# mnigm2001/Software-Defined-Radio

Hardware: AMD Instinct MI355X
Metric: I/Q MS/s through front-end FIR+decimate+demod(+audio) per job; % HBM roofline (higher is better)
Workload: dtype i8+f32

## Files before the change

### software-defined-radio_amd/csrc/kernels_fe_mfma.hip

```cpp
#include "device_math.hpp"
#include "fe_mfma_host.hpp"
#include "fmrx_internal.hpp"

#include <cmath>
#include <type_traits>
#include <utility>

namespace fmrx {
namespace {

using i4 = int __attribute__((ext_vector_type(4)));
using f2 = float __attribute__((ext_vector_type(2)));
using f4 = float __attribute__((ext_vector_type(4)));

constexpr int kNtPolicy = 2;

constexpr int iclamp(int v, int lo, int hi) { return v < lo ? lo : (v > hi ? hi : v); }
constexpr int igcd(int a, int b) { return b == 0 ? a : igcd(b, a % b); }

template <int T, int D, int PF = 0>
struct MfCfg {
    static constexpr int COL_OUT = 8;
    static constexpr int COLS = 16;
    static constexpr int TILE_OUT = COL_OUT * (COLS - 1);
// ... 210 lines not shown
        for (int d = 0; d < C::NDIG; d++) acc[d] = (i4){0, 0, 0, 0};
#pragma unroll
        for (int j = 0; j < C::KSTEPS; j++) {
            const i4 bs = b[j] ^ static_cast<int>(0x80808080u);
#pragma unroll
            for (int d = 0; d < C::NDIG; d++) acc[d] = __builtin_amdgcn_mfma_i32_16x16x64_i8(a[j][d], bs, acc[d], 0, 0, 0);
        }

        float v[4];
#pragma unroll
        for (int k = 0; k < 4; k++) {
            int lo = acc[0][k];
            if (C::NDIG >= 2) lo += acc[1][k] * 256;
            const float flo = static_cast<float>(lo) * scale_lo;
            v[k] = C::NDIG >= 3 ? __builtin_fmaf(static_cast<float>(acc[2][k]), scale_hi, flo) : flo;
        }
        float pi = __shfl(v[2], src_lane, 64), pq = __shfl(v[3], src_lane, 64);
        const long o = static_cast<long>(tile) * C::TILE_OUT + C::COL_OUT * (col - 1) + 2 * g;
        if (override_prev && o == 0) {
            pi = ovi;
            pq = ovq;
        }
        float d0 = 0.0f, d1 = 0.0f;
        if (demod) {
            d0 = demod_fast(v[0], v[1], pi, pq);
            d1 = demod_fast(v[2], v[3], v[0], v[1]);
        }

        if (col > 0 && o < n_out) {
            if (o + 1 < n_out) {
                if (demod) *reinterpret_cast<f2 *>(demod + o) = (f2){d0, d1};
                if (with_if) *reinterpret_cast<f4 *>(y_if + 2 * o) = (f4){v[0], v[1], v[2], v[3]};
                if (prev_out && o + 2 == n_out) *prev_out = make_float2(v[2], v[3]);
            } else {
                if (demod) demod[o] = d0;
                if (with_if) *reinterpret_cast<f2 *>(y_if + 2 * o) = (f2){v[0], v[1]};
                if (prev_out) *prev_out = make_float2(v[0], v[1]);
            }
        }
        slot = slot + 1 == C::NSLOT ? 0 : slot + 1;
        fill = fill + 1 == C::NSLOT ? 0 : fill + 1;
    }
}

template <int T, int D, int MINB = 2, int PF = 0>
int launch_mfma(const FePlan &pl, const uint8_t *d_iq, size_t n_samples, const uint8_t *d_hist, const float *d_prev,
                float *d_demod, float *d_if, float *d_prev_out, uint8_t *d_hist_next, hipStream_t stream,
                const float *d_dhist_src = nullptr, float *d_dhist_dst = nullptr, int dhist_n = 0)
{
    using C = MfCfg<T, D, PF>;
    if (C::LEAD > pl.hist_bytes) return fail(FMRX_EINVAL, "fe_mfma: history too short");
    const long n_out = static_cast<long>(n_samples / D);
    const long n_tiles = (n_out + C::TILE_OUT - 1) / C::TILE_OUT;
    long wgs_per_cu = (160 * 1024) / (4L * C::RING);
    if (wgs_per_cu > MINB) wgs_per_cu = MINB;
    const long want = (n_tiles + 3) / 4;
    const long grid = want < 256 * wgs_per_cu ? want : 256 * wgs_per_cu;
    hipLaunchKernelGGL((fe_mfma_kernel<T, D, MINB, PF>), dim3(static_cast<unsigned>(grid)), dim3(256), 4 * C::RING, stream, d_iq,
                       d_hist + pl.hist_bytes, static_cast<long>(2 * n_samples), reinterpret_cast<const i4 *>(pl.a_img.p),
                       pl.scale_lo, reinterpret_cast<const float2 *>(d_prev), d_demod, d_if,
                       reinterpret_cast<float2 *>(d_prev_out), n_out, static_cast<int>(n_tiles), d_hist_next, pl.hist_bytes,
                       d_dhist_src, d_dhist_dst, dhist_n);
    hipError_t e = hipGetLastError();
    if (e != hipSuccess) return fail(FMRX_EHIP, "launch fe_mfma_kernel<%d,%d>: %s", T, D, hipGetErrorString(e));
    return FMRX_OK;
}

struct FeBankGeom {
    long in_pitch, in_off;
    long out_pitch, out_off;
    long n_row;
    int tiles_per_row;
};

template <int T, int D>
__global__ __launch_bounds__(256, 2) void fe_mfma_bank_kernel(const uint8_t *__restrict__ x, long n_bytes, const i4 *__restrict__ a_img,
                                                               float scale_lo, float *__restrict__ demod, FeBankGeom bk, int n_tiles)
{
    using C = MfCfg<T, D, 0>;
    extern __shared__ __attribute__((aligned(16))) uint8_t lds_raw[];
    const int lane = threadIdx.x & 63;
    const int wave = __builtin_amdgcn_readfirstlane(static_cast<int>(threadIdx.x >> 6));
    uint8_t *ring = lds_raw + wave * C::RING;
    const int tstep = static_cast<int>(gridDim.x) * 4;
    int tile = __builtin_amdgcn_readfirstlane(static_cast<int>(blockIdx.x) * 4 + wave);
    if (tile >= n_tiles) return;
    i4 a[C::KSTEPS][C::NDIG];
#pragma unroll
    for (int j = 0; j < C::KSTEPS; j++)
#pragma unroll
        for (int d = 0; d < C::NDIG; d++) a[j][d] = a_img[(j * C::NDIG + d) * 64 + lane];
    asm volatile("s_waitcnt vmcnt(0)" ::: "memory");
#pragma unroll
    for (int j = 0; j < C::KSTEPS; j++)
#pragma unroll
        for (int d = 0; d < C::NDIG; d++) asm volatile("" : "+v"(a[j][d]));
    auto dma = [&](int t, int rs) {
        const int c = t / bk.tiles_per_row, j = t - c * bk.tiles_per_row;
        const long s0 = c * bk.in_pitch + bk.in_off + static_cast<long>(j) * C::STRIDE_BYTES - C::LEAD;
        dma_window<C::NPF, C::REM_LANES>(x, x, n_bytes, s0, ring + rs * C::SLOT, lane);
    };
#pragma unroll
    for (int k = 0; k < C::P; k++)
        if (tile + k * tstep < n_tiles) dma(tile + k * tstep, k);
    const int col = lane & 15, g = lane >> 4;
    const int lane_off = C::COL_BYTES * col + 16 * g;
    const float scale_hi = scale_lo * 65536.0f;
    const int src_lane = lane >= 16 ? lane - 16 : lane + 47;
    int slot = 0, fill = C::P;
    for (int it = 0; tile < n_tiles; tile += tstep, it++) {
        const bool steady = tile + C::P * tstep < n_tiles;
        if (steady) dma(tile + C::P * tstep, fill);
        if (steady) {
            if (it < C::P) wait_vmcnt<C::YOUNGER>();
            else wait_vmcnt<C::YOUNGER + C::P>();
        } else {
            wait_vmcnt<0>();
        }
        __builtin_amdgcn_fence(__ATOMIC_ACQUIRE, "wavefront");
        __builtin_amdgcn_wave_barrier();
        const uint8_t *bsrc = ring + slot * C::SLOT + lane_off;
        i4 b[C::KSTEPS];
#pragma unroll
        for (int j = 0; j < C::KSTEPS; j++) b[j] = *reinterpret_cast<const i4 *>(bsrc + 64 * j);
        __builtin_amdgcn_s_waitcnt(0xC07F);
        __builtin_amdgcn_fence(__ATOMIC_RELEASE, "wavefront");
        __builtin_amdgcn_wave_barrier();
        i4 acc[C::NDIG];
#pragma unroll
        for (int d = 0; d < C::NDIG; d++) acc[d] = (i4){0, 0, 0, 0};
#pragma unroll
        for (int j = 0; j < C::KSTEPS; j++) {
            const i4 bs = b[j] ^ static_cast<int>(0x80808080u);
#pragma unroll
            for (int d = 0; d < C::NDIG; d++) acc[d] = __builtin_amdgcn_mfma_i32_16x16x64_i8(a[j][d], bs, acc[d], 0, 0, 0);
        }
        float v[4];
#pragma unroll
        for (int k = 0; k < 4; k++) {
            int lo = acc[0][k];
            if (C::NDIG >= 2) lo += acc[1][k] * 256;
            const float flo = static_cast<float>(lo) * scale_lo;
            v[k] = C::NDIG >= 3 ? __builtin_fmaf(static_cast<float>(acc[2][k]), scale_hi, flo) : flo;
        }
        const float pi = __shfl(v[2], src_lane, 64), pq = __shfl(v[3], src_lane, 64);
        const float d0 = demod_fast(v[0], v[1], pi, pq), d1 = demod_fast(v[2], v[3], v[0], v[1]);
        const int c = tile / bk.tiles_per_row, j = tile - c * bk.tiles_per_row;
        const long ol = static_cast<long>(j) * C::TILE_OUT + C::COL_OUT * (col - 1) + 2 * g;
        if (col > 0 && ol < bk.n_row) *reinterpret_cast<f2 *>(demod + c * bk.out_pitch + bk.out_off + ol) = (f2){d0, d1};
        slot = slot + 1 == C::NSLOT ? 0 : slot + 1;
        fill = fill + 1 == C::NSLOT ? 0 : fill + 1;
    }
}

template <int T, int D, int TA, int DA>
struct FuCfg {
    using F = MfCfg<T, D>;
    static constexpr int TILE_OUT = 128;
    static constexpr int TILE_BYTES = F::COL_BYTES * 16;
    static constexpr int NPF = TILE_BYTES / 1024;
    static constexpr int REM_LANES = (TILE_BYTES % 1024) / 16;
    static constexpr int NP = NPF + (REM_LANES ? 1 : 0);
    static constexpr int P = iclamp(6144 / TILE_BYTES, 2, 8);
    static constexpr int NSLOT = P + 2;
    static constexpr int RING = NSLOT * TILE_BYTES;
    static constexpr int PIECE0 = NPF ? 1024 : TILE_BYTES;
    static_assert(F::WIN - F::COL_BYTES <= PIECE0, "window overlap must fit the next slot's first piece");
    static_assert(64 * F::KSTEPS - F::COL_BYTES <= RING - TILE_BYTES, "K padding laps the ring");
    static constexpr int YOUNGER = (NP - 1) + NP * P;
    static_assert(YOUNGER <= 63, "vmcnt is 6 bits");
    static constexpr int AB_OUT = 256;
    static constexpr int TB = AB_OUT * DA / TILE_OUT;
    static_assert(TB * TILE_OUT == AB_OUT * DA, "batches end on tile boundaries");
    static constexpr int SLOT_STEP = igcd(TB, NSLOT);
    static constexpr int NSTART = NSLOT / SLOT_STEP;
    static constexpr int LANE_OFF_END = F::COL_BYTES * (F::COLS - 1) + 16 * 3 + 16;
    static constexpr int AWIN = (TA - 1) + 15 * DA + 1;
    static constexpr int AK = (AWIN + 15) / 16 * 4;
    static_assert(AK % 4 == 0 && (TA - 1) % 4 == 0, "window in whole 16-byte groups");
    static constexpr int KPT = ((AK + TB - 3) / (TB - 2) + 3) / 4 * 4;
    static constexpr int NPH = (AK + KPT - 1) / KPT;
    static constexpr int DR_MIN = AB_OUT * DA + TA - 1 + (4 * AK - AWIN) + (NPH + 1) * TILE_OUT;
    static constexpr int DR = (DR_MIN + TILE_OUT - 1) / TILE_OUT * TILE_OUT;
    static_assert(NPH <= TB - 2, "a batch must be done before the next one completes");
    static_assert(AB_OUT * DA + TA - 1 + (4 * AK - AWIN) + (NPH + 1) * TILE_OUT <= DR, "ring too small for the delayed multiply");
    static_assert(DR % TILE_OUT == 0, "tiles must not wrap inside");
    static_assert(TA - 1 <= TILE_OUT - 1, "one dry tile must cover the audio history");
    static constexpr int MIRROR = 4 * KPT;
    static_assert(MIRROR <= TILE_OUT, "the mirror is refreshed by the tile at position 0");
    static constexpr int LDS_WAVE = RING + (DR + MIRROR) * 4;
};

template <class C, class F>
__device__ __forceinline__ void fu_dma_slot(const uint8_t *__restrict__ x, const uint8_t *__restrict__ hist_end, long n_bytes,
                                            int u, uint8_t *ring, int rs, int lane)
{
    dma_window<C::NPF, C::REM_LANES, kNtPolicy>(x, hist_end, n_bytes, static_cast<long>(u) * C::TILE_BYTES - F::FRONT,
                                                ring + rs * C::TILE_BYTES, lane);
}

template <int T, int D, int TA, int DA>
__global__ __launch_bounds__(256, 2) void mono_fused_kernel(
    const uint8_t *__restrict__ x, const uint8_t *__restrict__ hist_end, long n_bytes, const i4 *__restrict__ a_img,
    float scale_lo, const float *__restrict__ au_img, const float2 *__restrict__ prev_in,
    const float *__restrict__ dhist_end, float *__restrict__ demod_tail, int tail_keep, float2 *__restrict__ prev_out,
    float *__restrict__ audio, int16_t *__restrict__ pcm, int wrap, long n_out, int n_tiles, long n_audio, int n_batches,
    int batches_per_wave, uint8_t *__restrict__ hist_next, int hist_bytes)
{
    using C = FuCfg<T, D, TA, DA>;
    using F = typename C::F;
    extern __shared__ __attribute__((aligned(16))) uint8_t lds_raw[];
    const int lane = threadIdx.x & 63;
    const int wave = __builtin_amdgcn_readfirstlane(static_cast<int>(threadIdx.x >> 6));
    uint8_t *ring = lds_raw + wave * C::LDS_WAVE;
    float *dring = reinterpret_cast<float *>(ring + C::RING);
    const int wid = __builtin_amdgcn_readfirstlane(static_cast<int>(blockIdx.x) * 4 + wave);

    if (hist_next && wid == 0)
        for (int i = lane; i < hist_bytes; i += 64) hist_next[i] = x[n_bytes - hist_bytes + i];

    const int b0 = wid * batches_per_wave;
    const int b1 = b0 + batches_per_wave < n_batches ? b0 + batches_per_wave : n_batches;
    if (b0 >= b1) return;
    const int t0 = b0 * C::TB;
    const int t1 = b1 * C::TB < n_tiles ? b1 * C::TB : n_tiles;
    const int tb = t0 > 0 ? t0 - 1 : 0;

    i4 a[F::KSTEPS][F::NDIG];
#pragma unroll
    for (int j = 0; j < F::KSTEPS; j++)
#pragma unroll
        for (int d = 0; d < F::NDIG; d++) a[j][d] = a_img[(j * F::NDIG + d) * 64 + lane];
    float au[C::AK];
#pragma unroll
    for (int j = 0; j < C::AK; j++) au[j] = au_img[j * 64 + lane];
    float ci = 0.0f, cq = 0.0f;
    for (int i = lane; i < C::DR + C::MIRROR; i += 64) dring[i] = 0.0f;
    if (t0 == 0) {
        const float2 p = *prev_in;
        ci = p.x;
        cq = p.y;
        for (int i = lane; i < TA - 1; i += 64) dring[C::TILE_OUT - (TA - 1) + i] = dhist_end[i - (TA - 1)];
    }
    asm volatile("s_waitcnt vmcnt(0) lgkmcnt(0)" ::: "memory");
#pragma unroll
    for (int j = 0; j < F::KSTEPS; j++)
#pragma unroll
        for (int d = 0; d < F::NDIG; d++) asm volatile("" : "+v"(a[j][d]));
#pragma unroll
    for (int j = 0; j < C::AK; j++) asm volatile("" : "+v"(au[j]));
    asm volatile("" : "+v"(ci), "+v"(cq));

    for (int u = tb; u <= tb + C::P && u <= t1; u++) fu_dma_slot<C, F>(x, hist_end, n_bytes, u, ring, u % C::NSLOT, lane);

    const int col = lane & 15, g = lane >> 4;
    const int lane_off = F::COL_BYTES * col + 16 * g;
    const float scale_hi = scale_lo * 65536.0f;
    const int src_lane = lane >= 16 ? lane - 16 : lane + 47;
    int wrap_adr[F::KSTEPS];
#pragma unroll
    for (int j = 0; j < F::KSTEPS; j++) {
        const int adr = (C::NSLOT - 1) * C::TILE_BYTES + lane_off + 64 * j;
        wrap_adr[j] = adr >= C::RING ? adr - C::RING : adr;
    }
    int slot = tb % C::NSLOT, fill = (tb + C::P + 1) % C::NSLOT;
    int dpos = C::TILE_OUT;
    bool pend = false;
    int pend_ph = 0, pend_ws = 0;
    long pend_a0 = 0;
    f4 y0 = (f4){0.0f, 0.0f, 0.0f, 0.0f}, y1 = y0;
    f4 xs[C::KPT / 4];
    auto slice_load = [&]() {
#pragma unroll
        for (int k = 0; k < C::KPT / 4; k++)
            xs[k] = *reinterpret_cast<const f4 *>(dring + pend_ws + 16 * k);
        pend_ws += 4 * C::KPT;
        pend_ws = pend_ws >= C::DR ? pend_ws - C::DR : pend_ws;
    };
    auto slice_mfma = [&]() {
#pragma unroll
        for (int ph = 0; ph < C::NPH; ph++)
            if (pend_ph == ph) {
#pragma unroll
                for (int j = ph * C::KPT; j < (ph + 1) * C::KPT && j < C::AK; j++) {
                    const float xv = xs[(j - ph * C::KPT) / 4][j % 4];
                    if (j & 1) y1 = __builtin_amdgcn_mfma_f32_16x16x4f32(au[j], xv, y1, 0, 0, 0);
                    else y0 = __builtin_amdgcn_mfma_f32_16x16x4f32(au[j], xv, y0, 0, 0, 0);
                }
            }
    };
    auto store_batch = [&]() {
        const f4 y = y0 + y1;
        const long ao = pend_a0 + 4 * g;
        if (ao + 3 < n_audio) {
            if (audio) *reinterpret_cast<f4 *>(audio + ao) = y;
            if (pcm) {
                using s4 = short __attribute__((ext_vector_type(4)));
                const s4 pk = (s4){pcm_pack_flat(y[0], wrap), pcm_pack_flat(y[1], wrap), pcm_pack_flat(y[2], wrap), pcm_pack_flat(y[3], wrap)};
                *reinterpret_cast<s4 *>(pcm + ao) = pk;
            }
        } else {
#pragma unroll
            for (int k = 0; k < 4; k++)
                if (ao + k < n_audio) {
                    if (audio) audio[ao + k] = y[k];
                    if (pcm) pcm[ao + k] = pcm_pack(y[k], wrap);
                }
        }
    };
    auto slice_done = [&]() {
        pend_ph++;
        if (pend_ph == C::NPH) {
            store_batch();
            pend = false;
        }
    };
    auto begin_batch = [&](int bt) {
        pend = true;
        pend_ph = 0;
        pend_a0 = static_cast<long>(bt) * C::AB_OUT + 16 * col;
        int sb = (bt * C::AB_OUT * DA - (TA - 1)) - (C::TILE_OUT * tb - C::TILE_OUT);
        pend_ws = (sb + 16 * col * DA + 4 * g) % C::DR;
        y0 = (f4){0.0f, 0.0f, 0.0f, 0.0f};
        y1 = y0;
    };
    int t_fast1 = 0;
    bool fast_last = false;
    if (scale_lo >= 8.8817842e-16f) {
        const long in_x = (n_bytes - C::NP * 1024L + F::FRONT) / C::TILE_BYTES;
        const long no_tail = (n_out - tail_keep) / C::TILE_OUT - 1;
        long lim = t1 - C::P - 1;
        lim = lim < in_x - C::P - 1 ? lim : in_x - C::P - 1;
        lim = lim < no_tail ? lim : no_tail;
        t_fast1 = lim + 1 >= C::TB ? static_cast<int>((lim + 1) / C::TB) * C::TB : 0;
        fast_last = t1 % C::TB == 0 && t1 - C::TB >= t0 && t1 <= in_x && t1 - 1 <= no_tail;
    }
    int t_cur = tb;
    const long rbase = static_cast<long>(tb) * C::TILE_BYTES;
    const long reach = static_cast<long>(t1 - tb + 1) * C::TILE_BYTES + C::NP * 1024L;
    const __amdgpu_buffer_rsrc_t xr = __builtin_amdgcn_make_buffer_rsrc(
        const_cast<uint8_t *>(x + rbase), 0, static_cast<int>(reach < n_bytes - rbase ? reach : n_bytes - rbase), 0x00020000);
    const int lane16 = 16 * lane;
    const uint8_t *lring = ring + lane_off;
    auto fast_tile = [&](auto kc, auto lastc, auto sc, int t) {
        constexpr int k = decltype(kc)::value;
        constexpr int U = (decltype(sc)::value + k) % C::NSLOT;
        constexpr int FILL = (U + C::P + 1) % C::NSLOT;
        constexpr bool STEADY = !decltype(lastc)::value || k + C::P + 1 <= C::TB;
        constexpr int WAIT = STEADY ? C::YOUNGER : (C::NP - 1) + C::NP * (C::TB - k - 1);
        auto slice_k = [&]() {
#pragma unroll
            for (int j = k * C::KPT; j < (k + 1) * C::KPT && j < C::AK; j++) {
                const float xv = xs[(j - k * C::KPT) / 4][j % 4];
                if (j & 1) y1 = __builtin_amdgcn_mfma_f32_16x16x4f32(au[j], xv, y1, 0, 0, 0);
                else y0 = __builtin_amdgcn_mfma_f32_16x16x4f32(au[j], xv, y0, 0, 0, 0);
            }
        };
        if constexpr (STEADY) {
            const int soff = (t + C::P + 1 - tb) * C::TILE_BYTES - F::FRONT;
            for_each_index(std::make_integer_sequence<int, C::NP>{}, [&](auto qc) {
                constexpr int q = decltype(qc)::value;
                if (q < C::NPF || lane < C::REM_LANES)
                    __builtin_amdgcn_raw_ptr_buffer_load_lds(
                        xr, (__attribute__((address_space(3))) void *)(ring + FILL * C::TILE_BYTES + q * 1024), 16, lane16,
                        soff + q * 1024, 0, kNtPolicy);
            });
        }
        wait_vmcnt<WAIT>();
        __builtin_amdgcn_fence(__ATOMIC_ACQUIRE, "wavefront");
        __builtin_amdgcn_wave_barrier();
        i4 b[F::KSTEPS];
        for_each_index(std::make_integer_sequence<int, F::KSTEPS>{}, [&](auto jc) {
            constexpr int j = decltype(jc)::value;
            constexpr int OFF = U * C::TILE_BYTES + 64 * j;
            if constexpr (OFF + C::LANE_OFF_END > C::RING) {
                static_assert(U == C::NSLOT - 1, "only the last slot wraps");
                b[j] = *reinterpret_cast<const i4 *>(ring + wrap_adr[j]);
            } else {
                b[j] = *reinterpret_cast<const i4 *>(lring + OFF);
            }
        });
        if constexpr (k < C::NPH) slice_load();
        __builtin_amdgcn_sched_barrier(0);
        __builtin_amdgcn_s_waitcnt(0xC07F);
        __builtin_amdgcn_fence(__ATOMIC_RELEASE, "wavefront");
        __builtin_amdgcn_wave_barrier();
        i4 acc[F::NDIG];
#pragma unroll
        for (int d = 0; d < F::NDIG; d++) acc[d] = (i4){0, 0, 0, 0};
#pragma unroll
        for (int j = 0; j < F::KSTEPS; j++) {
            const i4 bs = b[j] ^ static_cast<int>(0x80808080u);
#pragma unroll
            for (int d = 0; d < F::NDIG; d++) acc[d] = __builtin_amdgcn_mfma_i32_16x16x64_i8(a[j][d], bs, acc[d], 0, 0, 0);
        }
        float v[4];
#pragma unroll
        for (int q = 0; q < 4; q++) {
            int lo = acc[0][q];
            if (F::NDIG >= 2) lo += acc[1][q] * 256;
            const float flo = static_cast<float>(lo) * scale_lo;
            v[q] = F::NDIG >= 3 ? __builtin_fmaf(static_cast<float>(acc[2][q]), scale_hi, flo) : flo;
        }
        float pi = __shfl(v[2], src_lane, 64), pq = __shfl(v[3], src_lane, 64);
        pi = lane == 0 ? ci : pi;
        pq = lane == 0 ? cq : pq;
        ci = __builtin_bit_cast(float, __builtin_amdgcn_readlane(__builtin_bit_cast(int, v[2]), 63));
        cq = __builtin_bit_cast(float, __builtin_amdgcn_readlane(__builtin_bit_cast(int, v[3]), 63));
        const float d0 = demod_fast_bounded(v[0], v[1], pi, pq);
        const float d1 = demod_fast_bounded(v[2], v[3], v[0], v[1]);
        const int ol = F::COL_OUT * col + 2 * g;
        *reinterpret_cast<f2 *>(dring + dpos + ol) = (f2){d0, d1};
        if (dpos == 0 && ol < C::MIRROR) *reinterpret_cast<f2 *>(dring + C::DR + ol) = (f2){d0, d1};
        dpos = dpos + C::TILE_OUT == C::DR ? 0 : dpos + C::TILE_OUT;
        if constexpr (k < C::NPH) slice_k();
        if constexpr (k == C::NPH - 1) store_batch();
    };
    auto fast_batch = [&](auto lastc) {
        const int s0 = t_cur % C::NSLOT;
        for_each_index(std::make_integer_sequence<int, C::NSTART>{}, [&](auto ic) {
            constexpr int S = decltype(ic)::value * C::SLOT_STEP;
            if (s0 == S)
                for_each_index(std::make_integer_sequence<int, C::TB>{}, [&](auto kc) {
                    fast_tile(kc, lastc, std::integral_constant<int, S>{}, t_cur + decltype(kc)::value);
                });
        });
        begin_batch(t_cur / C::TB);
        t_cur += C::TB;
    };
    for (int &t = t_cur;;) {
        if (t >= t0 && (t < t_fast1 || (fast_last && t == t1 - C::TB)) && t % C::TB == 0 && (!pend || pend_ph == 0)) {
            if (!pend) {
                begin_batch(t / C::TB);
                pend_a0 = n_audio;
            }
            while (t < t_fast1) fast_batch(std::false_type{});
            if (fast_last && t == t1 - C::TB) fast_batch(std::true_type{});
            slot = t % C::NSLOT;
            fill = (t + C::P + 1) % C::NSLOT;
        }
        const bool have_tile = t < t1;
        bool completed = false;
        if (have_tile) {
            const bool sl = pend;
            const bool steady = t + C::P + 1 <= t1;
            if (steady) fu_dma_slot<C, F>(x, hist_end, n_bytes, t + C::P + 1, ring, fill, lane);
            if (steady) wait_vmcnt<C::YOUNGER>();
            else wait_vmcnt<0>();
            __builtin_amdgcn_fence(__ATOMIC_ACQUIRE, "wavefront");
            __builtin_amdgcn_wave_barrier();

            i4 b[F::KSTEPS];
            if (slot != C::NSLOT - 1) {
                const uint8_t *bsrc = ring + slot * C::TILE_BYTES + lane_off;
#pragma unroll
                for (int j = 0; j < F::KSTEPS; j++) b[j] = *reinterpret_cast<const i4 *>(bsrc + 64 * j);
            } else {
#pragma unroll
                for (int j = 0; j < F::KSTEPS; j++) b[j] = *reinterpret_cast<const i4 *>(ring + wrap_adr[j]);
            }
            if (sl) slice_load();
            __builtin_amdgcn_s_waitcnt(0xC07F);
            __builtin_amdgcn_fence(__ATOMIC_RELEASE, "wavefront");
            __builtin_amdgcn_wave_barrier();

            i4 acc[F::NDIG];
#pragma unroll
            for (int d = 0; d < F::NDIG; d++) acc[d] = (i4){0, 0, 0, 0};
#pragma unroll
            for (int j = 0; j < F::KSTEPS; j++) {
                const i4 bs = b[j] ^ static_cast<int>(0x80808080u);
#pragma unroll
                for (int d = 0; d < F::NDIG; d++)
                    acc[d] = __builtin_amdgcn_mfma_i32_16x16x64_i8(a[j][d], bs, acc[d], 0, 0, 0);
            }
            float v[4];
#pragma unroll
            for (int k = 0; k < 4; k++) {
                int lo = acc[0][k];
                if (F::NDIG >= 2) lo += acc[1][k] * 256;
                const float flo = static_cast<float>(lo) * scale_lo;
                v[k] = F::NDIG >= 3 ? __builtin_fmaf(static_cast<float>(acc[2][k]), scale_hi, flo) : flo;
            }
            float pi = __shfl(v[2], src_lane, 64), pq = __shfl(v[3], src_lane, 64);
            if (lane == 0) {
                pi = ci;
                pq = cq;
            }
            ci = __builtin_bit_cast(float, __builtin_amdgcn_readlane(__builtin_bit_cast(int, v[2]), 63));
            cq = __builtin_bit_cast(float, __builtin_amdgcn_readlane(__builtin_bit_cast(int, v[3]), 63));
            const float d0 = demod_fast(v[0], v[1], pi, pq);
            const float d1 = demod_fast(v[2], v[3], v[0], v[1]);

            const int ol = F::COL_OUT * col + 2 * g;
            const long o = static_cast<long>(t) * C::TILE_OUT + ol;
            *reinterpret_cast<f2 *>(dring + dpos + ol) = (f2){d0, d1};
            if (dpos == 0 && ol < C::MIRROR) *reinterpret_cast<f2 *>(dring + C::DR + ol) = (f2){d0, d1};
            if (t >= t0 && static_cast<long>(t + 1) * C::TILE_OUT > n_out - tail_keep &&
                o + 2 > n_out - tail_keep && o < n_out) {
                if (demod_tail && o >= n_out - tail_keep) demod_tail[o] = d0;
                if (demod_tail && o + 1 < n_out) demod_tail[o + 1] = d1;
                if (prev_out && o + 2 == n_out) *prev_out = make_float2(v[2], v[3]);
                if (prev_out && o + 1 == n_out) *prev_out = make_float2(v[0], v[1]);
            }
            slot = slot + 1 == C::NSLOT ? 0 : slot + 1;
            fill = fill + 1 == C::NSLOT ? 0 : fill + 1;
            dpos = dpos + C::TILE_OUT == C::DR ? 0 : dpos + C::TILE_OUT;
            if (sl) {
                slice_mfma();
                slice_done();
            }
            completed = t >= t0 && ((t + 1) % C::TB == 0 || t + 1 == n_tiles);
            t++;
        }

        while (pend && (completed || !have_tile)) {
            slice_load();
            slice_mfma();
            slice_done();
        }
        if (completed) begin_batch((t - 1) / C::TB);
        if (!have_tile && !pend) break;
    }
}

template <int T, int D, int TA, int DA>
int launch_fused_mono(const FePlan &fe, const AudioPlan &au, const uint8_t *d_iq, size_t n_samples, const uint8_t *d_hist,
                      const float *d_prev, const float *d_dhist_end, float *d_demod_tail, int tail_keep, float *d_prev_out,
                      float *d_audio, int16_t *d_pcm, int wrap, uint8_t *d_hist_next, hipStream_t stream)
{
    using C = FuCfg<T, D, TA, DA>;
    if (C::F::FRONT > fe.hist_bytes) return fail(FMRX_EINVAL, "mono_fused: history too short");
    const long n_out = static_cast<long>(n_samples / D);
    const long n_tiles = (n_out + C::TILE_OUT - 1) / C::TILE_OUT;
    const long n_audio = n_out / DA;
    const long n_batches = (n_audio + C::AB_OUT - 1) / C::AB_OUT;
    long wgs_per_cu = (160 * 1024) / (4L * C::LDS_WAVE);
    if (wgs_per_cu > 2) wgs_per_cu = 2;
    const int lds_bytes = 4 * C::LDS_WAVE;
    const long max_waves = 256 * wgs_per_cu * 4;
    const long bpw = (n_batches + max_waves - 1) / max_waves;
    const long grid = ((n_batches + bpw - 1) / bpw + 3) / 4;
    if (lds_bytes > 64 * 1024) {
        static bool raised[64] = {};
        int dev = 0;
        FMRX_HIP(hipGetDevice(&dev));
        if (dev < 0 || dev >= 64 || !raised[dev]) {
            FMRX_HIP(hipFuncSetAttribute(reinterpret_cast<const void *>(&mono_fused_kernel<T, D, TA, DA>),
                                         hipFuncAttributeMaxDynamicSharedMemorySize, lds_bytes));
            if (dev >= 0 && dev < 64) raised[dev] = true;
        }
    }
    hipLaunchKernelGGL((mono_fused_kernel<T, D, TA, DA>), dim3(static_cast<unsigned>(grid)), dim3(256), lds_bytes, stream,
                       d_iq, d_hist + fe.hist_bytes, static_cast<long>(2 * n_samples), reinterpret_cast<const i4 *>(fe.a_img.p),
                       fe.scale_lo, au.mfma_table.p, reinterpret_cast<const float2 *>(d_prev), d_dhist_end, d_demod_tail,
                       tail_keep, reinterpret_cast<float2 *>(d_prev_out), d_audio, d_pcm, wrap, n_out, static_cast<int>(n_tiles),
                       n_audio, static_cast<int>(n_batches), static_cast<int>(bpw), d_hist_next, fe.hist_bytes);
    hipError_t e = hipGetLastError();
    if (e != hipSuccess)
        return fail(FMRX_EHIP, "launch mono_fused_kernel<%d,%d,%d,%d>: %s", T, D, TA, DA, hipGetErrorString(e));
    return FMRX_OK;
}

#define FMRX_FUSED_CASES(X)                                                                         \
    X(101, 10, 101, 5) X(151, 10, 101, 5) X(13, 10, 101, 5) X(101, 10, 13, 5) X(151, 10, 13, 5) X(13, 10, 13, 5) \
    X(101, 5, 101, 6) X(151, 5, 101, 6) X(13, 5, 101, 6) X(101, 5, 13, 6) X(151, 5, 13, 6) X(13, 5, 13, 6)

#define FMRX_FE_MFMA_CASES(X) X(13, 10) X(101, 10) X(151, 10) X(13, 5) X(101, 5) X(151, 5) X(13, 3) X(101, 3) X(151, 3)

}

int fe_mfma_plan_init(FePlan &pl, const float *h, int taps, int decim)
{
    pl.mfma = false;
    int s = 0;
    if (!fe_mfma_scale(h, taps, kFeMfmaDigits, &s)) return FMRX_OK;
    std::vector<int8_t> img;
#define X(T_, D_)                                                                          \
    if (taps == T_ && decim == D_) {                                                       \
        static_assert(MfCfg<T_, D_>::NDIG == kFeMfmaDigits, "digit count");                \
        if (fe_mfma_shape(T_, D_).ksteps != MfCfg<T_, D_>::KSTEPS || fe_mfma_shape(T_, D_).front != MfCfg<T_, D_>::FRONT) \
            return fail(FMRX_EINVAL, "fe_mfma: host and device tile shapes disagree");     \
        fe_mfma_build_image(h, T_, D_, s, kFeMfmaDigits, img);                             \
        pl.mfma = true;                                                                    \
    }
    FMRX_FE_MFMA_CASES(X)
#undef X
    if (!pl.mfma) return FMRX_OK;
    pl.scale_lo = static_cast<float>(std::ldexp(1.0, -s - 7));
    FMRX_TRY(pl.silence.alloc(pl.hist_bytes));
    FMRX_HIP(hipMemset(pl.silence.p, 128, pl.hist_bytes));
    FMRX_TRY(pl.a_img.alloc((img.size() + 3) / 4));
    FMRX_HIP(hipMemcpy(pl.a_img.p, img.data(), img.size(), hipMemcpyHostToDevice));
    return FMRX_OK;
}

bool fe_mfma_available(const FePlan &pl, const uint8_t *d_iq, size_t n_samples, const uint8_t *d_hist)
{
    return pl.mfma && d_hist && n_samples >= 8 && (reinterpret_cast<uintptr_t>(d_iq) % 16 == 0) &&
           ((2 * n_samples) % 16 == 0) && (reinterpret_cast<uintptr_t>(d_hist) % 16 == 0) && pl.hist_bytes % 16 == 0;
}

int fe_mfma_launch(const FePlan &pl, const uint8_t *d_iq, size_t n_samples, const uint8_t *d_hist, const float *d_prev,
                   float *d_demod, float *d_if, float *d_prev_out, uint8_t *d_hist_next, const Options &o, hipStream_t stream,
                   const float *d_dhist_src, float *d_dhist_dst, int dhist_n)
{
    if (n_samples / pl.decim == 0) return FMRX_OK;
    if (!d_demod && !d_if) return fail(FMRX_EINVAL, "fe_mfma_launch: no output");
#define X(T_, D_) \
    if (pl.taps == T_ && pl.decim == D_) \
        return launch_mfma<T_, D_, (T_ <= 101 && D_ == 3) ? 3 : (T_ <= 101 && D_ == 5) ? 4 : 2, \
                           (T_ <= 101 && D_ == 3) ? 4 : (T_ <= 101 && D_ == 5) ? 2 : 0>( \
            pl, d_iq, n_samples, d_hist, d_prev, d_demod, d_if, d_prev_out, d_hist_next, stream, d_dhist_src, d_dhist_dst, dhist_n);
    FMRX_FE_MFMA_CASES(X)
#undef X
    return fail(FMRX_EINVAL, "fe_mfma_launch: no kernel for taps=%d decim=%d", pl.taps, pl.decim);
}

int fe_mfma_bank_lead(const FePlan &pl)
{
#define X(T_, D_) if (pl.taps == T_ && pl.decim == D_) return MfCfg<T_, D_>::LEAD;
    FMRX_FE_MFMA_CASES(X)
#undef X
    return -1;
}

int fe_mfma_bank_launch(const FePlan &pl, const uint8_t *d_slots, long total_bytes, long in_pitch, long block_off, int n_channels,
                        long k_lo, long k_hi, float *d_demod, long out_pitch, long out_off, hipStream_t stream)
{
    if (!pl.mfma) return fail(FMRX_EINVAL, "fe_mfma_bank: no matrix-core kernel for taps=%d decim=%d", pl.taps, pl.decim);
    if ((k_hi - k_lo) % 2 || (k_lo * pl.decim * 2) % 16 || in_pitch % 16 || block_off % 16 || out_pitch % 2 || (out_off + k_lo) % 2)
        return fail(FMRX_EINVAL, "fe_mfma_bank: misaligned geometry");
#define X(T_, D_)                                                                                                             \
    if (pl.taps == T_ && pl.decim == D_) {                                                                                    \
        using C = MfCfg<T_, D_>;                                                                                              \
        FeBankGeom bk;                                                                                                        \
        bk.in_pitch = in_pitch;                                                                                               \
        bk.in_off = block_off + k_lo * D_ * 2;                                                                                \
        bk.out_pitch = out_pitch;                                                                                             \
        bk.out_off = out_off + k_lo;                                                                                          \
        bk.n_row = k_hi - k_lo;                                                                                               \
        bk.tiles_per_row = static_cast<int>((bk.n_row + C::TILE_OUT - 1) / C::TILE_OUT);                                      \
        const long n_tiles = static_cast<long>(bk.tiles_per_row) * n_channels;                                                \
        if (n_tiles > 0x7fffffffL / 4) return fail(FMRX_EINVAL, "fe_mfma_bank: too many tiles");                              \
        const long want = (n_tiles + 3) / 4;                                                                                  \
        const long grid = want < 256 ? want : 256;                                                                            \
        hipLaunchKernelGGL((fe_mfma_bank_kernel<T_, D_>), dim3(static_cast<unsigned>(grid)), dim3(256), 4 * C::RING, stream,  \
                           d_slots, total_bytes, reinterpret_cast<const i4 *>(pl.a_img.p), pl.scale_lo, d_demod, bk,         \
                           static_cast<int>(n_tiles));                                                                        \
        hipError_t e = hipGetLastError();                                                                                     \
        if (e != hipSuccess) return fail(FMRX_EHIP, "launch fe_mfma_bank_kernel<%d,%d>: %s", T_, D_, hipGetErrorString(e)); \
        return FMRX_OK;                                                                                                       \
    }
    FMRX_FE_MFMA_CASES(X)
#undef X
    return fail(FMRX_EINVAL, "fe_mfma_bank: no kernel for taps=%d decim=%d", pl.taps, pl.decim);
}

int audio_mfma_table_init(AudioPlan &pl, const float *h, int taps, int decim)
{
    std::vector<float> tab;
    audio_mfma_build_table(h, taps, decim, tab);
    FMRX_TRY(pl.mfma_table.alloc(tab.size()));
    FMRX_HIP(hipMemcpy(pl.mfma_table.p, tab.data(), tab.size() * sizeof(float), hipMemcpyHostToDevice));
    return FMRX_OK;
}

bool mono_fused_available(const FePlan &fe, const AudioPlan &au, const uint8_t *d_iq, size_t n_samples, const uint8_t *d_hist)
{
    if (!fe_mfma_available(fe, d_iq, n_samples, d_hist) || !au.mfma_table.p) return false;
    for (int k = 0; k < 1; k++) {
#define X(T_, D_, TA_, DA_) \
    if (fe.taps == T_ && fe.decim == D_ && au.taps == TA_ && au.decim == DA_) return true;
        FMRX_FUSED_CASES(X)
#undef X
    }
    return false;
}

int mono_fused_launch(const FePlan &fe, const AudioPlan &au, const uint8_t *d_iq, size_t n_samples, const uint8_t *d_hist,
                      const float *d_prev, const float *d_dhist_end, float *d_demod_tail, int tail_keep, float *d_prev_out,
                      float *d_audio, int16_t *d_pcm, int wrap, uint8_t *d_hist_next, const Options &o, hipStream_t stream)
{
    if (!d_prev || !d_dhist_end) return fail(FMRX_EINVAL, "mono_fused_launch: null argument");
#define X(T_, D_, TA_, DA_)                                                                                          \
    if (fe.taps == T_ && fe.decim == D_ && au.taps == TA_ && au.decim == DA_)                                         \
        return launch_fused_mono<T_, D_, TA_, DA_>(fe, au, d_iq, n_samples, d_hist, d_prev, d_dhist_end, d_demod_tail, \
                                                   tail_keep, d_prev_out, d_audio, d_pcm, wrap, d_hist_next, stream);
    FMRX_FUSED_CASES(X)
#undef X
    return fail(FMRX_EINVAL, "mono_fused_launch: no kernel for this filter shape");
}

}
```

Before: 2.712 million.

## Split fused kernel into stream waves and dedicated audio-filter waves synchronized by barriers

The fused mono kernel is reorganized into warp specialization: four stream waves run the front-end FIR, decimation and demodulation into their LDS demod rings, and two extra waves per workgroup each run the audio FIR multiply for two stream waves. Hand-off uses workgroup barriers at half-batch and full-batch boundaries, replacing the interleaved sliced audio multiply inside the stream loop. The aim is to take the audio MFMA work and the au registers off the stream waves' critical path. In exchange it adds s_barrier synchronization, a bigger demod ring, different occupancy (6-wave blocks, launch bounds of 3) and a risk of barrier-count mismatches between waves.

```diff
diff --git a/software-defined-radio_amd/csrc/kernels_fe_mfma.hip b/software-defined-radio_amd/csrc/kernels_fe_mfma.hip
--- a/software-defined-radio_amd/csrc/kernels_fe_mfma.hip
+++ b/software-defined-radio_amd/csrc/kernels_fe_mfma.hip
@@ -386,6 +386,9 @@
         fill = fill + 1 == C::NSLOT ? 0 : fill + 1;
     }
 }
+
+constexpr int kFuStreamWaves = 4;
+constexpr int kFuWaves = kFuStreamWaves + kFuStreamWaves / 2;
 
 template <int T, int D, int TA, int DA>
 struct FuCfg {
@@ -412,16 +415,16 @@
     static constexpr int AWIN = (TA - 1) + 15 * DA + 1;
     static constexpr int AK = (AWIN + 15) / 16 * 4;
     static_assert(AK % 4 == 0 && (TA - 1) % 4 == 0, "window in whole 16-byte groups");
-    static constexpr int KPT = ((AK + TB - 3) / (TB - 2) + 3) / 4 * 4;
-    static constexpr int NPH = (AK + KPT - 1) / KPT;
-    static constexpr int DR_MIN = AB_OUT * DA + TA - 1 + (4 * AK - AWIN) + (NPH + 1) * TILE_OUT;
+    static constexpr int SW = kFuStreamWaves, AW = SW / 2, WAVES = kFuWaves;
+    static_assert(TB % 2 == 0, "the half-batch barrier stands on a tile boundary");
+    static constexpr int HB = TB / 2;
+    static constexpr int DR_MIN = (1 + TB + HB) * TILE_OUT + (4 * AK - AWIN);
     static constexpr int DR = (DR_MIN + TILE_OUT - 1) / TILE_OUT * TILE_OUT;
-    static_assert(NPH <= TB - 2, "a batch must be done before the next one completes");
-    static_assert(AB_OUT * DA + TA - 1 + (4 * AK - AWIN) + (NPH + 1) * TILE_OUT <= DR, "ring too small for the delayed multiply");
+    static_assert((1 + TB + HB) * TILE_OUT + (4 * AK - AWIN) <= DR, "ring too small for the hand-off");
     static_assert(DR % TILE_OUT == 0, "tiles must not wrap inside");
     static_assert(TA - 1 <= TILE_OUT - 1, "one dry tile must cover the audio history");
-    static constexpr int MIRROR = 4 * KPT;
-    static_assert(MIRROR <= TILE_OUT, "the mirror is refreshed by the tile at position 0");
+    static constexpr int MIRROR = 4 * AK;
+    static_assert(MIRROR <= 2 * TILE_OUT && MIRROR <= DR, "the mirror is refreshed by the tiles at positions 0 and TILE_OUT");
     static constexpr int LDS_WAVE = RING + (DR + MIRROR) * 4;
 };
 
@@ -434,7 +437,7 @@
 }
 
 template <int T, int D, int TA, int DA>
-__global__ __launch_bounds__(256, 2) void mono_fused_kernel(
+__global__ __launch_bounds__(kFuWaves * 64, 3) void mono_fused_kernel(
     const uint8_t *__restrict__ x, const uint8_t *__restrict__ hist_end, long n_bytes, const i4 *__restrict__ a_img,
     float scale_lo, const float *__restrict__ au_img, const float2 *__restrict__ prev_in,
     const float *__restrict__ dhist_end, float *__restrict__ demod_tail, int tail_keep, float2 *__restrict__ prev_out,
@@ -446,16 +449,114 @@
     extern __shared__ __attribute__((aligned(16))) uint8_t lds_raw[];
     const int lane = threadIdx.x & 63;
     const int wave = __builtin_amdgcn_readfirstlane(static_cast<int>(threadIdx.x >> 6));
+    const int col = lane & 15, g = lane >> 4;
+    auto wg_barrier = [&]() {
+        asm volatile("" ::: "memory");
+        __builtin_amdgcn_s_waitcnt(0xC07F);
+        __builtin_amdgcn_s_barrier();
+        asm volatile("" ::: "memory");
+    };
+
+    if (wave >= C::SW) {
+        float au[C::AK];
+#pragma unroll
+        for (int j = 0; j < C::AK; j++) au[j] = au_img[j * 64 + lane];
+        const float *win[2];
+        long a0[2];
+        int left[2];
+        int wstep[2];
+#pragma unroll
+        for (int s = 0; s < 2; s++) {
+            const int sw = 2 * (wave - C::SW) + s;
+            const int swid = static_cast<int>(blockIdx.x) * C::SW + sw;
+            const int sb0 = swid * batches_per_wave;
+            const int sb1 = sb0 + batches_per_wave < n_batches ? sb0 + batches_per_wave : n_batches;
+            const int st0 = sb0 * C::TB;
+            const int stb = st0 > 0 ? st0 - 1 : 0;
+            left[s] = sb1 > sb0 ? sb1 - sb0 : 0;
+            const int sb = (sb0 * C::AB_OUT * DA - (TA - 1)) - (C::TILE_OUT * stb - C::TILE_OUT);
+            wstep[s] = (sb + 16 * col * DA + 4 * g) % C::DR;
+            win[s] = reinterpret_cast<const float *>(lds_raw + sw * C::LDS_WAVE + C::RING);
+            a0[s] = static_cast<long>(sb0) * C::AB_OUT + 16 * col;
+        }
+        auto store_batch = [&](const f4 y, const long ao16) {
+            const long ao = ao16 + 4 * g;
+            if (ao + 3 < n_audio) {
+                if (audio) *reinterpret_cast<f4 *>(audio + ao) = y;
+                if (pcm) {
+                    using s4 = short __attribute__((ext_vector_type(4)));
+                    const s4 pk = (s4){pcm_pack_flat(y[0], wrap), pcm_pack_flat(y[1], wrap), pcm_pack_flat(y[2], wrap), pcm_pack_flat(y[3], wrap)};
+                    *reinterpret_cast<s4 *>(pcm + ao) = pk;
+                }
+            } else {
+#pragma unroll
+                for (int k = 0; k < 4; k++)
+                    if (ao + k < n_audio) {
+                        if (audio) audio[ao + k] = y[k];
+                        if (pcm) pcm[ao + k] = pcm_pack(y[k], wrap);
+                    }
+            }
+        };
+        auto multiply = [&](auto firstc, auto nc) {
+            constexpr int FIRST = decltype(firstc)::value, N = decltype(nc)::value;
+            f4 y0[N], y1[N];
+#pragma unroll
+            for (int s = 0; s < N; s++) {
+                y0[s] = (f4){0.0f, 0.0f, 0.0f, 0.0f};
+                y1[s] = y0[s];
+            }
+#pragma unroll
+            for (int k = 0; k < C::AK / 4; k++) {
+                f4 xs[N];
+#pragma unroll
+                for (int s = 0; s < N; s++)
+                    xs[s] = *reinterpret_cast<const f4 *>(win[FIRST + s] + wstep[FIRST + s] + 16 * k);
+#pragma unroll
+                for (int q = 0; q < 4; q++)
+#pragma unroll
+                    for (int s = 0; s < N; s++) {
+                        if (q & 1) y1[s] = __builtin_amdgcn_mfma_f32_16x16x4f32(au[4 * k + q], xs[s][q], y1[s], 0, 0, 0);
+                        else y0[s] = __builtin_amdgcn_mfma_f32_16x16x4f32(au[4 * k + q], xs[s][q], y0[s], 0, 0, 0);
+                    }
+            }
+#pragma unroll
+            for (int s = 0; s < N; s++) {
+                store_batch(y0[s] + y1[s], a0[FIRST + s]);
+                a0[FIRST + s] += C::AB_OUT;
+                wstep[FIRST + s] += C::AB_OUT * DA;
+                wstep[FIRST + s] = wstep[FIRST + s] >= C::DR ? wstep[FIRST + s] - C::DR : wstep[FIRST + s];
+                left[FIRST + s]--;
+            }
+        };
+        wg_barrier();
+        for (int i = 0; i <= batches_per_wave; i++) {
+            if (i > 0) {
+                using I0 = std::integral_constant<int, 0>;
+                using I1 = std::integral_constant<int, 1>;
+                using I2 = std::integral_constant<int, 2>;
+                if (left[0] > 0 && left[1] > 0) multiply(I0{}, I2{});
+                else if (left[0] > 0) multiply(I0{}, I1{});
+                else if (left[1] > 0) multiply(I1{}, I1{});
+            }
+            wg_barrier();
+            wg_barrier();
+        }
+        return;
+    }
+
     uint8_t *ring = lds_raw + wave * C::LDS_WAVE;
     float *dring = reinterpret_cast<float *>(ring + C::RING);
-    const int wid = __builtin_amdgcn_readfirstlane(static_cast<int>(blockIdx.x) * 4 + wave);
+    const int wid = __builtin_amdgcn_readfirstlane(static_cast<int>(blockIdx.x) * C::SW + wave);
 
     if (hist_next && wid == 0)
         for (int i = lane; i < hist_bytes; i += 64) hist_next[i] = x[n_bytes - hist_bytes + i];
 
     const int b0 = wid * batches_per_wave;
     const int b1 = b0 + batches_per_wave < n_batches ? b0 + batches_per_wave : n_batches;
-    if (b0 >= b1) return;
+    if (b0 >= b1) {
+        for (int i = 0; i < 2 * batches_per_wave + 3; i++) wg_barrier();
+        return;
+    }
     const int t0 = b0 * C::TB;
     const int t1 = b1 * C::TB < n_tiles ? b1 * C::TB : n_tiles;
     const int tb = t0 > 0 ? t0 - 1 : 0;
@@ -465,9 +566,6 @@
     for (int j = 0; j < F::KSTEPS; j++)
 #pragma unroll
         for (int d = 0; d < F::NDIG; d++) a[j][d] = a_img[(j * F::NDIG + d) * 64 + lane];
-    float au[C::AK];
-#pragma unroll
-    for (int j = 0; j < C::AK; j++) au[j] = au_img[j * 64 + lane];
     float ci = 0.0f, cq = 0.0f;
     for (int i = lane; i < C::DR + C::MIRROR; i += 64) dring[i] = 0.0f;
     if (t0 == 0) {
@@ -481,13 +579,10 @@
     for (int j = 0; j < F::KSTEPS; j++)
 #pragma unroll
         for (int d = 0; d < F::NDIG; d++) asm volatile("" : "+v"(a[j][d]));
-#pragma unroll
-    for (int j = 0; j < C::AK; j++) asm volatile("" : "+v"(au[j]));
     asm volatile("" : "+v"(ci), "+v"(cq));
 
     for (int u = tb; u <= tb + C::P && u <= t1; u++) fu_dma_slot<C, F>(x, hist_end, n_bytes, u, ring, u % C::NSLOT, lane);
 
-    const int col = lane & 15, g = lane >> 4;
     const int lane_off = F::COL_BYTES * col + 16 * g;
     const float scale_hi = scale_lo * 65536.0f;
     const int src_lane = lane >= 16 ? lane - 16 : lane + 47;
@@ -497,66 +592,12 @@
         const int adr = (C::NSLOT - 1) * C::TILE_BYTES + lane_off + 64 * j;
         wrap_adr[j] = adr >= C::RING ? adr - C::RING : adr;
     }
-    int slot = tb % C::NSLOT, fill = (tb + C::P + 1) % C::NSLOT;
     int dpos = C::TILE_OUT;
-    bool pend = false;
-    int pend_ph = 0, pend_ws = 0;
-    long pend_a0 = 0;
-    f4 y0 = (f4){0.0f, 0.0f, 0.0f, 0.0f}, y1 = y0;
-    f4 xs[C::KPT / 4];
-    auto slice_load = [&]() {
-#pragma unroll
-        for (int k = 0; k < C::KPT / 4; k++)
-            xs[k] = *reinterpret_cast<const f4 *>(dring + pend_ws + 16 * k);
-        pend_ws += 4 * C::KPT;
-        pend_ws = pend_ws >= C::DR ? pend_ws - C::DR : pend_ws;
-    };
-    auto slice_mfma = [&]() {
-#pragma unroll
-        for (int ph = 0; ph < C::NPH; ph++)
-            if (pend_ph == ph) {
-#pragma unroll
-                for (int j = ph * C::KPT; j < (ph + 1) * C::KPT && j < C::AK; j++) {
-                    const float xv = xs[(j - ph * C::KPT) / 4][j % 4];
-                    if (j & 1) y1 = __builtin_amdgcn_mfma_f32_16x16x4f32(au[j], xv, y1, 0, 0, 0);
-                    else y0 = __builtin_amdgcn_mfma_f32_16x16x4f32(au[j], xv, y0, 0, 0, 0);
-                }
-            }
-    };
-    auto store_batch = [&]() {
-        const f4 y = y0 + y1;
-        const long ao = pend_a0 + 4 * g;
-        if (ao + 3 < n_audio) {
-            if (audio) *reinterpret_cast<f4 *>(audio + ao) = y;
-            if (pcm) {
-                using s4 = short __attribute__((ext_vector_type(4)));
-                const s4 pk = (s4){pcm_pack_flat(y[0], wrap), pcm_pack_flat(y[1], wrap), pcm_pack_flat(y[2], wrap), pcm_pack_flat(y[3], wrap)};
-                *reinterpret_cast<s4 *>(pcm + ao) = pk;
-            }
-        } else {
-#pragma unroll
-            for (int k = 0; k < 4; k++)
-                if (ao + k < n_audio) {
-                    if (audio) audio[ao + k] = y[k];
-                    if (pcm) pcm[ao + k] = pcm_pack(y[k], wrap);
-                }
-        }
-    };
-    auto slice_done = [&]() {
-        pend_ph++;
-        if (pend_ph == C::NPH) {
-            store_batch();
-            pend = false;
-        }
-    };
-    auto begin_batch = [&](int bt) {
-        pend = true;
-        pend_ph = 0;
-        pend_a0 = static_cast<long>(bt) * C::AB_OUT + 16 * col;
-        int sb = (bt * C::AB_OUT * DA - (TA - 1)) - (C::TILE_OUT * tb - C::TILE_OUT);
-        pend_ws = (sb + 16 * col * DA + 4 * g) % C::DR;
-        y0 = (f4){0.0f, 0.0f, 0.0f, 0.0f};
-        y1 = y0;
+    const int ol = F::COL_OUT * col + 2 * g;
+    auto ring_write = [&](const float d0, const float d1) {
+        *reinterpret_cast<f2 *>(dring + dpos + ol) = (f2){d0, d1};
+        if (dpos < C::MIRROR && dpos + ol < C::MIRROR) *reinterpret_cast<f2 *>(dring + C::DR + dpos + ol) = (f2){d0, d1};
+        dpos = dpos + C::TILE_OUT == C::DR ? 0 : dpos + C::TILE_OUT;
     };
     int t_fast1 = 0;
     bool fast_last = false;
@@ -569,7 +610,6 @@
         t_fast1 = lim + 1 >= C::TB ? static_cast<int>((lim + 1) / C::TB) * C::TB : 0;
         fast_last = t1 % C::TB == 0 && t1 - C::TB >= t0 && t1 <= in_x && t1 - 1 <= no_tail;
     }
-    int t_cur = tb;
     const long rbase = static_cast<long>(tb) * C::TILE_BYTES;
     const long reach = static_cast<long>(t1 - tb + 1) * C::TILE_BYTES + C::NP * 1024L;
     const __amdgpu_buffer_rsrc_t xr = __builtin_amdgcn_make_buffer_rsrc(
@@ -582,14 +622,6 @@
         constexpr int FILL = (U + C::P + 1) % C::NSLOT;
         constexpr bool STEADY = !decltype(lastc)::value || k + C::P + 1 <= C::TB;
         constexpr int WAIT = STEADY ? C::YOUNGER : (C::NP - 1) + C::NP * (C::TB - k - 1);
-        auto slice_k = [&]() {
-#pragma unroll
-            for (int j = k * C::KPT; j < (k + 1) * C::KPT && j < C::AK; j++) {
-                const float xv = xs[(j - k * C::KPT) / 4][j % 4];
-                if (j & 1) y1 = __builtin_amdgcn_mfma_f32_16x16x4f32(au[j], xv, y1, 0, 0, 0);
-                else y0 = __builtin_amdgcn_mfma_f32_16x16x4f32(au[j], xv, y0, 0, 0, 0);
-            }
-        };
         if constexpr (STEADY) {
             const int soff = (t + C::P + 1 - tb) * C::TILE_BYTES - F::FRONT;
             for_each_index(std::make_integer_sequence<int, C::NP>{}, [&](auto qc) {
@@ -600,6 +632,7 @@
                         soff + q * 1024, 0, kNtPolicy);
             });
         }
+        if constexpr (k == C::HB) wg_barrier();
         wait_vmcnt<WAIT>();
         __builtin_amdgcn_fence(__ATOMIC_ACQUIRE, "wavefront");
         __builtin_amdgcn_wave_barrier();
@@ -614,7 +647,6 @@
                 b[j] = *reinterpret_cast<const i4 *>(lring + OFF);
             }
         });
-        if constexpr (k < C::NPH) slice_load();
         __builtin_amdgcn_sched_barrier(0);
         __builtin_amdgcn_s_waitcnt(0xC07F);
         __builtin_amdgcn_fence(__ATOMIC_RELEASE, "wavefront");
@@ -643,118 +675,101 @@
         cq = __builtin_bit_cast(float, __builtin_amdgcn_readlane(__builtin_bit_cast(int, v[3]), 63));
         const float d0 = demod_fast_bounded(v[0], v[1], pi, pq);
         const float d1 = demod_fast_bounded(v[2], v[3], v[0], v[1]);
-        const int ol = F::COL_OUT * col + 2 * g;
-        *reinterpret_cast<f2 *>(dring + dpos + ol) = (f2){d0, d1};
-        if (dpos == 0 && ol < C::MIRROR) *reinterpret_cast<f2 *>(dring + C::DR + ol) = (f2){d0, d1};
-        dpos = dpos + C::TILE_OUT == C::DR ? 0 : dpos + C::TILE_OUT;
-        if constexpr (k < C::NPH) slice_k();
-        if constexpr (k == C::NPH - 1) store_batch();
+        ring_write(d0, d1);
+        if constexpr (k == C::TB - 1) wg_barrier();
     };
-    auto fast_batch = [&](auto lastc) {
-        const int s0 = t_cur % C::NSLOT;
+    auto fast_batch = [&](auto lastc, int t) {
+        const int s0 = t % C::NSLOT;
         for_each_index(std::make_integer_sequence<int, C::NSTART>{}, [&](auto ic) {
             constexpr int S = decltype(ic)::value * C::SLOT_STEP;
             if (s0 == S)
                 for_each_index(std::make_integer_sequence<int, C::TB>{}, [&](auto kc) {
-                    fast_tile(kc, lastc, std::integral_constant<int, S>{}, t_cur + decltype(kc)::value);
+                    fast_tile(kc, lastc, std::integral_constant<int, S>{}, t + decltype(kc)::value);
                 });
         });
-        begin_batch(t_cur / C::TB);
-        t_cur += C::TB;
     };
-    for (int &t = t_cur;;) {
-        if (t >= t0 && (t < t_fast1 || (fast_last && t == t1 - C::TB)) && t % C::TB == 0 && (!pend || pend_ph == 0)) {
-            if (!pend) {
-                begin_batch(t / C::TB);
-                pend_a0 = n_audio;
+    auto general_tile = [&](int t) {
+        const int slot = t % C::NSLOT, fill = (t + C::P + 1) % C::NSLOT;
+        const bool steady = t + C::P + 1 <= t1;
+        if (steady) fu_dma_slot<C, F>(x, hist_end, n_bytes, t + C::P + 1, ring, fill, lane);
+        if (steady) wait_vmcnt<C::YOUNGER>();
+        else wait_vmcnt<0>();
+        __builtin_amdgcn_fence(__ATOMIC_ACQUIRE, "wavefront");
+        __builtin_amdgcn_wave_barrier();
+
+        i4 b[F::KSTEPS];
+        if (slot != C::NSLOT - 1) {
+            const uint8_t *bsrc = ring + slot * C::TILE_BYTES + lane_off;
+#pragma unroll
+            for (int j = 0; j < F::KSTEPS; j++) b[j] = *reinterpret_cast<const i4 *>(bsrc + 64 * j);
+        } else {
+#pragma unroll
+            for (int j = 0; j < F::KSTEPS; j++) b[j] = *reinterpret_cast<const i4 *>(ring + wrap_adr[j]);
+        }
+        __builtin_amdgcn_s_waitcnt(0xC07F);
+        __builtin_amdgcn_fence(__ATOMIC_RELEASE, "wavefront");
+        __builtin_amdgcn_wave_barrier();
+
+        i4 acc[F::NDIG];
+#pragma unroll
+        for (int d = 0; d < F::NDIG; d++) acc[d] = (i4){0, 0, 0, 0};
+#pragma unroll
+        for (int j = 0; j < F::KSTEPS; j++) {
+            const i4 bs = b[j] ^ static_cast<int>(0x80808080u);
+#pragma unroll
+            for (int d = 0; d < F::NDIG; d++)
+                acc[d] = __builtin_amdgcn_mfma_i32_16x16x64_i8(a[j][d], bs, acc[d], 0, 0, 0);
+        }
+        float v[4];
+#pragma unroll
+        for (int k = 0; k < 4; k++) {
+            int lo = acc[0][k];
+            if (F::NDIG >= 2) lo += acc[1][k] * 256;
+            const float flo = static_cast<float>(lo) * scale_lo;
+            v[k] = F::NDIG >= 3 ? __builtin_fmaf(static_cast<float>(acc[2][k]), scale_hi, flo) : flo;
+        }
+        float pi = __shfl(v[2], src_lane, 64), pq = __shfl(v[3], src_lane, 64);
+        if (lane == 0) {
+            pi = ci;
+            pq = cq;
+        }
+        ci = __builtin_bit_cast(float, __builtin_amdgcn_readlane(__builtin_bit_cast(int, v[2]), 63));
+        cq = __builtin_bit_cast(float, __builtin_amdgcn_readlane(__builtin_bit_cast(int, v[3]), 63));
+        const float d0 = demod_fast(v[0], v[1], pi, pq);
+        const float d1 = demod_fast(v[2], v[3], v[0], v[1]);
+
+        const long o = static_cast<long>(t) * C::TILE_OUT + ol;
+        ring_write(d0, d1);
+        if (t >= t0 && static_cast<long>(t + 1) * C::TILE_OUT > n_out - tail_keep &&
+            o + 2 > n_out - tail_keep && o < n_out) {
+            if (demod_tail && o >= n_out - tail_keep) demod_tail[o] = d0;
+            if (demod_tail && o + 1 < n_out) demod_tail[o + 1] = d1;
+            if (prev_out && o + 2 == n_out) *prev_out = make_float2(v[2], v[3]);
+            if (prev_out && o + 1 == n_out) *prev_out = make_float2(v[0], v[1]);
+        }
+    };
+
+    if (tb < t0) general_tile(tb);
+    wg_barrier();
+    for (int i = 0; i <= batches_per_wave; i++) {
+        const int t = (b0 + i) * C::TB;
+        if (i < batches_per_wave && t < t1) {
+            if (t < t_fast1) {
+                fast_batch(std::false_type{}, t);
+            } else if (fast_last && t == t1 - C::TB) {
+                fast_batch(std::true_type{}, t);
+            } else {
+#pragma unroll 1
+                for (int k = 0; k < C::TB; k++) {
+                    if (k == C::HB) wg_barrier();
+                    if (t + k < t1) general_tile(t + k);
+                }
+                wg_barrier();
             }
-            while (t < t_fast1) fast_batch(std::false_type{});
-            if (fast_last && t == t1 - C::TB) fast_batch(std::true_type{});
-            slot = t % C::NSLOT;
-            fill = (t + C::P + 1) % C::NSLOT;
-        }
-        const bool have_tile = t < t1;
-        bool completed = false;
-        if (have_tile) {
-            const bool sl = pend;
-            const bool steady = t + C::P + 1 <= t1;
-            if (steady) fu_dma_slot<C, F>(x, hist_end, n_bytes, t + C::P + 1, ring, fill, lane);
-            if (steady) wait_vmcnt<C::YOUNGER>();
-            else wait_vmcnt<0>();
-            __builtin_amdgcn_fence(__ATOMIC_ACQUIRE, "wavefront");
-            __builtin_amdgcn_wave_barrier();
-
-            i4 b[F::KSTEPS];
-            if (slot != C::NSLOT - 1) {
-                const uint8_t *bsrc = ring + slot * C::TILE_BYTES + lane_off;
-#pragma unroll
-                for (int j = 0; j < F::KSTEPS; j++) b[j] = *reinterpret_cast<const i4 *>(bsrc + 64 * j);
-            } else {
-#pragma unroll
-                for (int j = 0; j < F::KSTEPS; j++) b[j] = *reinterpret_cast<const i4 *>(ring + wrap_adr[j]);
-            }
-            if (sl) slice_load();
-            __builtin_amdgcn_s_waitcnt(0xC07F);
-            __builtin_amdgcn_fence(__ATOMIC_RELEASE, "wavefront");
-            __builtin_amdgcn_wave_barrier();
-
-            i4 acc[F::NDIG];
-#pragma unroll
-            for (int d = 0; d < F::NDIG; d++) acc[d] = (i4){0, 0, 0, 0};
-#pragma unroll
-            for (int j = 0; j < F::KSTEPS; j++) {
-                const i4 bs = b[j] ^ static_cast<int>(0x80808080u);
-#pragma unroll
-                for (int d = 0; d < F::NDIG; d++)
-                    acc[d] = __builtin_amdgcn_mfma_i32_16x16x64_i8(a[j][d], bs, acc[d], 0, 0, 0);
-            }
-            float v[4];
-#pragma unroll
-            for (int k = 0; k < 4; k++) {
-                int lo = acc[0][k];
-                if (F::NDIG >= 2) lo += acc[1][k] * 256;
-                const float flo = static_cast<float>(lo) * scale_lo;
-                v[k] = F::NDIG >= 3 ? __builtin_fmaf(static_cast<float>(acc[2][k]), scale_hi, flo) : flo;
-            }
-            float pi = __shfl(v[2], src_lane, 64), pq = __shfl(v[3], src_lane, 64);
-            if (lane == 0) {
-                pi = ci;
-                pq = cq;
-            }
-            ci = __builtin_bit_cast(float, __builtin_amdgcn_readlane(__builtin_bit_cast(int, v[2]), 63));
-            cq = __builtin_bit_cast(float, __builtin_amdgcn_readlane(__builtin_bit_cast(int, v[3]), 63));
-            const float d0 = demod_fast(v[0], v[1], pi, pq);
-            const float d1 = demod_fast(v[2], v[3], v[0], v[1]);
-
-            const int ol = F::COL_OUT * col + 2 * g;
-            const long o = static_cast<long>(t) * C::TILE_OUT + ol;
-            *reinterpret_cast<f2 *>(dring + dpos + ol) = (f2){d0, d1};
-            if (dpos == 0 && ol < C::MIRROR) *reinterpret_cast<f2 *>(dring + C::DR + ol) = (f2){d0, d1};
-            if (t >= t0 && static_cast<long>(t + 1) * C::TILE_OUT > n_out - tail_keep &&
-                o + 2 > n_out - tail_keep && o < n_out) {
-                if (demod_tail && o >= n_out - tail_keep) demod_tail[o] = d0;
-                if (demod_tail && o + 1 < n_out) demod_tail[o + 1] = d1;
-                if (prev_out && o + 2 == n_out) *prev_out = make_float2(v[2], v[3]);
-                if (prev_out && o + 1 == n_out) *prev_out = make_float2(v[0], v[1]);
-            }
-            slot = slot + 1 == C::NSLOT ? 0 : slot + 1;
-            fill = fill + 1 == C::NSLOT ? 0 : fill + 1;
-            dpos = dpos + C::TILE_OUT == C::DR ? 0 : dpos + C::TILE_OUT;
-            if (sl) {
-                slice_mfma();
-                slice_done();
-            }
-            completed = t >= t0 && ((t + 1) % C::TB == 0 || t + 1 == n_tiles);
-            t++;
-        }
-
-        while (pend && (completed || !have_tile)) {
-            slice_load();
-            slice_mfma();
-            slice_done();
-        }
-        if (completed) begin_batch((t - 1) / C::TB);
-        if (!have_tile && !pend) break;
+        } else {
+            wg_barrier();
+            wg_barrier();
+        }
     }
 }
 
@@ -769,12 +784,12 @@
     const long n_tiles = (n_out + C::TILE_OUT - 1) / C::TILE_OUT;
     const long n_audio = n_out / DA;
     const long n_batches = (n_audio + C::AB_OUT - 1) / C::AB_OUT;
-    long wgs_per_cu = (160 * 1024) / (4L * C::LDS_WAVE);
-    if (wgs_per_cu > 2) wgs_per_cu = 2;
-    const int lds_bytes = 4 * C::LDS_WAVE;
-    const long max_waves = 256 * wgs_per_cu * 4;
+    long wgs_per_cu = (160 * 1024) / (static_cast<long>(C::SW) * C::LDS_WAVE);
+    if (wgs_per_cu > 8 / C::SW) wgs_per_cu = 8 / C::SW;
+    const int lds_bytes = C::SW * C::LDS_WAVE;
+    const long max_waves = 256 * wgs_per_cu * C::SW;
     const long bpw = (n_batches + max_waves - 1) / max_waves;
-    const long grid = ((n_batches + bpw - 1) / bpw + 3) / 4;
+    const long grid = ((n_batches + bpw - 1) / bpw + C::SW - 1) / C::SW;
     if (lds_bytes > 64 * 1024) {
         static bool raised[64] = {};
         int dev = 0;
@@ -785,7 +800,7 @@
             if (dev >= 0 && dev < 64) raised[dev] = true;
         }
     }
-    hipLaunchKernelGGL((mono_fused_kernel<T, D, TA, DA>), dim3(static_cast<unsigned>(grid)), dim3(256), lds_bytes, stream,
+    hipLaunchKernelGGL((mono_fused_kernel<T, D, TA, DA>), dim3(static_cast<unsigned>(grid)), dim3(C::WAVES * 64), lds_bytes, stream,
                        d_iq, d_hist + fe.hist_bytes, static_cast<long>(2 * n_samples), reinterpret_cast<const i4 *>(fe.a_img.p),
                        fe.scale_lo, au.mfma_table.p, reinterpret_cast<const float2 *>(d_prev), d_dhist_end, d_demod_tail,
                        tail_keep, reinterpret_cast<float2 *>(d_prev_out), d_audio, d_pcm, wrap, n_out, static_cast<int>(n_tiles),
```

Result: slower. 2.291 million (-15.6%).
